# michaelneale/p2p-llm-tunnel

Measured on AMD Instinct MI355X. Metric: tunneled req/s + added p50 TTFT vs direct, mock-LLM SSE at 1/2/4/8 streams, higher is better.
Workload: dtype n/a

## Files before the change

p2p_llm_tunnel_amd/models/server.py:

```python
from __future__ import annotations

import argparse
import asyncio
import functools
import json
import os
import queue
import socket
import sys
import threading
import time
import uuid
from typing import NamedTuple

import torch


class Sampling:
    __slots__ = ("temperature", "top_k", "top_p", "seed")

    def __init__(self, temperature: float = 0.0, top_k: int = 0, top_p: float = 1.0, seed: int | None = None):
        self.temperature = float(temperature)
        self.top_k = int(top_k)
        self.top_p = float(top_p)
# ... 385 lines not shown
        self._pools = pools = []
        for r, row in enumerate(rows):
            s = self.slots[row.slot]
            if s["embed"]:
                if pools and pools[-1][0] == row.slot:
                    pools[-1][2] += 1
                else:
                    pools.append([row.slot, r, 1, row.pos == 0, None])
        max_seq = self.model.cfg.max_seq
        for row in rows:
            self.slots[row.slot]["pos"] += 1
            if not row.emit:
                self.prefill_tokens += 1
        done = []
        for r, row in enumerate(rows):
            if not row.emit:
                continue
            i = row.slot
            s = self.slots[i]
            s["gen"] += 1
            fin = s["gen"] >= s["req"].max_new or s["pos"] >= max_seq - 1
            emits.append((r, s["req"], fin, s["gen"] - 1))
            if fin:
                done.append(i)
        for pool in pools:
            s = self.slots[pool[0]]
            if s["pos"] >= len(s["ids"]):
                pool[4] = s["req"]
                done.append(pool[0])
        for i in done:
            self.slots[i] = None
        return rows, emits

    def _step_body(self, b: _StepBuf, n: int, run, sample_rows: int = 0, logprobs: bool = False):
        din = self._d_in[b.rows]
        din.copy_(b.h_in, non_blocking=True)
        d = din[:, :n]
        tok = torch.where(d[_DEC] != 0, self._d_last[d[_SLOT]], d[_TOK])
        ids, logits = run(tok, d[_POS].to(torch.int32), d[_SLOT].to(torch.int32))
        if sample_rows:
            from p2p_llm_tunnel_amd import ops
            ops.sample_(logits[:sample_rows], ids[:sample_rows], din[_SMP])
            if logprobs:
                ops.logprobs_(logits[:sample_rows], ids[:sample_rows], din[_LP], b.d_lp[:sample_rows],
                              b.d_lp_ids[:sample_rows])
                b.h_lp.copy_(b.d_lp, non_blocking=True)
                b.h_lp_ids.copy_(b.d_lp_ids, non_blocking=True)
        self._d_last.index_copy_(0, d[_REC], ids)
        b.h_out[:n].copy_(ids, non_blocking=True)

    def _capture(self, b: _StepBuf, emit_rows: int, post: int):
        from p2p_llm_tunnel_amd.models.tiny_llm import capture
        b.np[:] = 0
        b.np[_SLOT, :] = b.np[_REC, :] = self.model.scratch_slot
        run = functools.partial(self.model.step_rows, emit_rows=emit_rows)
        sample_rows = (emit_rows or b.rows) if post else 0
        graph, _ = capture(lambda: self._step_body(b, b.rows, run, sample_rows, post == 2), self.device)
        torch.cuda.synchronize(self.device)
        return graph

    def _launch(self, rows, emits) -> _StepBuf:
        n, scratch = len(rows), self.model.scratch_slot
        R = self.small_rows if self.use_graph and n <= self.small_rows else self.rows
        par = self._k % 2
        self._k += 1
        b = self._bufs[R][par]
        h = b.np
        h[_TOK, :n] = [r.token for r in rows]
        h[_POS, :n] = [r.pos for r in rows]
        h[_SLOT, :n] = [r.slot for r in rows]
        h[_DEC, :n] = [r.decode for r in rows]
        h[_REC, :n] = [r.slot if r.emit else scratch for r in rows]
        h[_SMP, :] = 0
        h[_LP, :] = 0
        post = 0
        for r, req, _, ctr in emits:
            if not req.sampling.greedy:
                h[_SMP, r] = req.sampling.column(ctr)
                post = max(post, 1)
            if req.logprobs is not None:
                h[_LP, r] = 1 + req.logprobs
                post = 2
        if n < R:
            h[_TOK, n:R] = h[_POS, n:R] = h[_DEC, n:R] = 0
            h[_SLOT, n:R] = h[_REC, n:R] = scratch
        b.n, b.emits = n, emits
        if self.use_graph:
            self._graphs[(R, par, post)].replay()
        else:
            rng = (min(r.pos for r in rows), max(r.pos for r in rows))
# ... 654 lines not shown
```

p2p_llm_tunnel_amd/models/tiny_llm.py:

```python
from __future__ import annotations

import math
from dataclasses import dataclass

import torch
import torch.nn.functional as F

from p2p_llm_tunnel_amd import ops


@dataclass(frozen=True)
class LlamaConfig:
    vocab: int = 32000
    dim: int = 1024
    n_layers: int = 4
    n_heads: int = 16
    n_kv_heads: int = 4
    head_dim: int = 64
    ffn: int = 2816
    max_seq: int = 2048
    eps: float = 1e-5
    rope_theta: float = 10000.0
    qk_norm: bool = False

# ... 111 lines not shown
            return torch.stack([torch.arange(n), torch.arange(n) + n], 1).flatten().to(self.device)

        heads = c.n_heads + 2 * c.n_kv_heads
        head_perm = (torch.arange(heads, device=self.device)[:, None] * c.head_dim
                     + pairs(c.head_dim // 2)[None, :]).flatten()
        ws = [self.embed, self.final_norm, fold(self.lm_head, self.final_norm)]
        for L in self.layers:
            wqkv = fold(L["wqkv"], L["attn_norm"])
            ws += [L["attn_norm"], wqkv.contiguous() if c.qk_norm else wqkv[head_perm].contiguous(), L["wo"],
                   L["ffn_norm"], fold(L["w_gate_up"], L["ffn_norm"])[pairs(c.ffn)].contiguous(), L["w_down"]]
            if c.qk_norm:
                ws += [L["q_norm"].contiguous(), L["k_norm"].contiguous()]
        return ws

    def fused_decoder(self) -> ops.FusedLlamaDecoder:
        if self._fused is None:
            c = self.cfg
            dims = ops.LlamaDims(vocab=c.vocab, dim=c.dim, n_layers=c.n_layers, H=c.n_heads, Hkv=c.n_kv_heads,
                                 D=c.head_dim, ffn=c.ffn, max_seq=c.max_seq, max_batch=self.max_batch + 1, eps=c.eps,
                                 theta=c.rope_theta, qk_norm=int(c.qk_norm))
            self._fused = ops.FusedLlamaDecoder(dims, self.fused_weights(), self.k_cache, self.v_cache)
        return self._fused

    def step_rows(self, tokens, pos, slots=None, emit_rows=0, pos_range=None):
        B = tokens.shape[0]
        if self.fused and B <= ops.MAX_ROWS:
            tokens, pos = tokens.contiguous(), pos.contiguous()
            slots = slots.contiguous() if slots is not None else None
            logits = torch.empty(B, self.cfg.vocab, dtype=torch.bfloat16, device=self.device)
            ids = torch.empty(B, dtype=torch.int64, device=self.device)
            self.fused_decoder().step(tokens, pos, logits, ids, slots, emit_rows)
            return ids, logits
        return self._decode_unfused(tokens, pos, pos_range or (0, self.cfg.max_seq - 1))

    def _decode_unfused(self, tokens, pos, pos_range):
        c = self.cfg
        B = tokens.shape[0]
        lens = pos + 1
        x = self.embed.index_select(0, tokens)
        h = ops.rmsnorm(x, self.layers[0]["attn_norm"], c.eps)
        residual = x
        for i, L in enumerate(self.layers):
            kc, vc = self.k_cache[i, :B], self.v_cache[i, :B]
            qkv = F.linear(h, L["wqkv"])
            if c.qk_norm:
                nq, nk = c.n_heads * c.head_dim, c.n_kv_heads * c.head_dim
                qn = ops.rmsnorm(qkv[:, :nq].reshape(-1, c.head_dim), L["q_norm"], c.eps).view(B, nq)
                kn = ops.rmsnorm(qkv[:, nq:nq + nk].reshape(-1, c.head_dim), L["k_norm"], c.eps).view(B, nk)
                qkv = torch.cat([qn, kn, qkv[:, nq + nk:]], 1)
            q = ops.rope_qkv_cache(qkv, pos, kc, vc, c.n_heads, c.n_kv_heads, c.head_dim, c.rope_theta,
                                   pos_range=pos_range)
            a = ops.decode_attention(q, kc, vc, lens, max_len=pos_range[1] + 1)
            o = F.linear(a.view(B, -1), L["wo"])
            h, residual = ops.rmsnorm(o, L["ffn_norm"], c.eps, residual=residual)
            m = F.linear(ops.silu_mul(F.linear(h, L["w_gate_up"])), L["w_down"])
            nxt = self.layers[i + 1]["attn_norm"] if i + 1 < len(self.layers) else self.final_norm
            h, residual = ops.rmsnorm(m, nxt, c.eps, residual=residual)
        logits = F.linear(h, self.lm_head)
        return ops.argmax(logits), logits

    def capture_graph(self, rows: int | None = None, emit_rows: int = 0):
        R = rows or (16 if self.fused else self.max_batch)
        g_tok = torch.zeros(R, dtype=torch.int64, device=self.device)
        g_pos = torch.zeros(R, dtype=torch.int32, device=self.device)
        g_slot = (torch.full((R,), self.scratch_slot, dtype=torch.int32, device=self.device)
                  if self.fused else None)
# ... 92 lines not shown
```

p2p_llm_tunnel_amd/ops/__init__.py:

```python
from __future__ import annotations

import ctypes
import math
import os

import torch

HERE = os.path.dirname(os.path.abspath(__file__))
_LIB = None


class LlamaDims(ctypes.Structure):
    _fields_ = [(n, ctypes.c_int) for n in ("vocab", "dim", "n_layers", "H", "Hkv", "D", "ffn", "max_seq",
                                           "max_batch")] + [("eps", ctypes.c_float), ("theta", ctypes.c_float),
                                                            ("qk_norm", ctypes.c_int)]


_INT = ctypes.c_int


class GemmPlan(ctypes.Structure):
    _fields_ = [(n, _INT) for n in ("epi", "nw", "tn", "um", "kpl", "grid_x", "grid_y", "ss_in", "M", "N", "K")]


class AttnPlan(ctypes.Structure):
    _fields_ = [(n, _INT) for n in ("D", "G", "slots", "stride", "grid_y")]


class StepPlan(ctypes.Structure):
    _fields_ = ([("rows", _INT), ("emit_rows", _INT)] +
                [(n, GemmPlan) for n in ("qkv_first", "qkv", "o", "gate_up", "down", "lm_head")] +
                [("attn", AttnPlan), ("am_parts", _INT), ("qk_norm_grid", _INT)])


def lib() -> ctypes.CDLL:
    global _LIB
    if _LIB is None:
        path = os.path.join(HERE, os.environ.get("P2PT_HIP_OPS_LIB", "_hip_ops.so"))
        if not os.path.exists(path):
            from . import build as _b
            _b.build()
        _LIB = ctypes.CDLL(path)
        vp, i, f = ctypes.c_void_p, ctypes.c_int, ctypes.c_float
        _LIB.p2pt_rmsnorm.argtypes = [vp, vp, vp, vp, vp, i, i, f, vp]
        _LIB.p2pt_silu_mul.argtypes = [vp, vp, i, i, vp]
        _LIB.p2pt_rope_qkv_cache.argtypes = [vp, vp, vp, vp, vp, i, i, i, i, i, f, vp]
        _LIB.p2pt_qk_norm_rope_cache.argtypes = [vp, vp, vp, vp, vp, vp, vp, vp, i, i, i, i, i, i, f, f, vp]
        _LIB.p2pt_decode_attention.argtypes = [vp, vp, vp, vp, vp, vp, i, i, i, i, i, i, i, f, vp]
        _LIB.p2pt_argmax.argtypes = [vp, vp, i, i, vp]
        _LIB.p2pt_skinny_gemm.argtypes = [vp, vp, vp, i, i, i, vp]
        _LIB.p2pt_sample.argtypes = [vp, vp, vp, i, i, i, vp]
        _LIB.p2pt_logprobs.argtypes = [vp, vp, vp, vp, vp, i, i, vp]
        _LIB.p2pt_kv_copy.argtypes = [vp, vp, i, i, i, i, i, ctypes.POINTER(ctypes.c_int), vp]
        _LIB.p2pt_max_kv_copy_jobs.argtypes = []
        _LIB.p2pt_embed_pool.argtypes = [vp, i, i, vp, vp, i, vp, i, f, i, ctypes.POINTER(ctypes.c_int), vp]
        _LIB.p2pt_max_embed_jobs.argtypes = []
        _LIB.p2pt_llama_ws_bytes.argtypes = [ctypes.POINTER(LlamaDims)]
        _LIB.p2pt_llama_ws_bytes.restype = ctypes.c_size_t
        szp = ctypes.POINTER(ctypes.c_size_t)
        _LIB.p2pt_llama_ws_layout.argtypes = [ctypes.POINTER(LlamaDims), szp, szp, i]
        _LIB.p2pt_llama_ws_layout.restype = ctypes.c_int
        _LIB.p2pt_llama_decode.argtypes = [ctypes.POINTER(LlamaDims), ctypes.POINTER(vp), vp, vp, vp, vp, vp, i, i,
                                           vp, ctypes.c_size_t, vp, vp, vp]
        _LIB.p2pt_llama_plan.argtypes = [ctypes.POINTER(LlamaDims), i, i, ctypes.POINTER(StepPlan)]
        _LIB.p2pt_attn_span.argtypes = [i, i]
        _LIB.p2pt_max_rows.argtypes = []
        _LIB.p2pt_skinny_bench.argtypes = [vp, vp, vp, i, i, i, i, i, i, vp]
        _LIB.p2pt_attn_bench.argtypes = [vp, vp, vp, vp, i, i, i, i, i, vp, vp, vp, vp, i, vp]
        for fn in ("p2pt_rmsnorm", "p2pt_silu_mul", "p2pt_rope_qkv_cache", "p2pt_decode_attention", "p2pt_argmax",
                   "p2pt_skinny_gemm", "p2pt_llama_decode", "p2pt_sample", "p2pt_logprobs", "p2pt_llama_plan", "p2pt_attn_span",
                   "p2pt_max_rows", "p2pt_skinny_bench", "p2pt_attn_bench", "p2pt_kv_copy", "p2pt_max_kv_copy_jobs",
                   "p2pt_embed_pool", "p2pt_max_embed_jobs", "p2pt_qk_norm_rope_cache"):
            getattr(_LIB, fn).restype = ctypes.c_int
        if _LIB.p2pt_max_rows() != MAX_ROWS:
            raise RuntimeError(f"MAX_ROWS = {MAX_ROWS}, but {path} was built for {_LIB.p2pt_max_rows()} rows")
        if _LIB.p2pt_max_kv_copy_jobs() != MAX_KV_COPY_JOBS:
            raise RuntimeError(f"MAX_KV_COPY_JOBS = {MAX_KV_COPY_JOBS}, but {path} was built for "
                               f"{_LIB.p2pt_max_kv_copy_jobs()} jobs")
        if _LIB.p2pt_max_embed_jobs() != MAX_EMBED_JOBS:
            raise RuntimeError(f"MAX_EMBED_JOBS = {MAX_EMBED_JOBS}, but {path} was built for "
                               f"{_LIB.p2pt_max_embed_jobs()} jobs")
    return _LIB


MAX_ROWS = 64
MAX_KV_COPY_JOBS = 8
MAX_EMBED_JOBS = 16
MAX_TOP_LOGPROBS = 20


def step_plan(dims: LlamaDims, B: int, emit_rows: int = 0) -> StepPlan:
    plan = StepPlan()
    if lib().p2pt_llama_plan(ctypes.byref(dims), B, emit_rows, ctypes.byref(plan)) != 0:
        raise ValueError("dims or row count not supported by the fused decode kernels")
    return plan


def attn_span(length: int, slots: int) -> int:
    return lib().p2pt_attn_span(length, slots)


def loaded_path() -> str:
    return lib()._name


# ... 162 lines not shown
        raise ValueError("lens exceed cache capacity")
    nsplit = max(1, math.ceil(max_len / chunk))
    ws = torch.empty(B * H * nsplit * (D + 2), dtype=torch.float32, device=q.device)
    out = torch.empty_like(q)
    scale = 1.0 / math.sqrt(D) if scale is None else scale
    _ok(lib().p2pt_decode_attention(_p(q), _p(k_cache), _p(v_cache), _p(lens), _p(out), _p(ws), B, H, Hkv, D, Smax,
                                    nsplit, chunk, scale, _stream(q)), "decode_attention")
    return out


def argmax(logits: torch.Tensor) -> torch.Tensor:
    _check(logits, torch.bfloat16, "logits")
    if logits.dim() != 2:
        raise ValueError("logits must be [B, V]")
    B, V = logits.shape
    out = torch.empty(B, dtype=torch.int64, device=logits.device)
    _ok(lib().p2pt_argmax(_p(logits), _p(out), B, V, _stream(logits)), "argmax")
    return out


def sample_(logits: torch.Tensor, ids: torch.Tensor, params: torch.Tensor) -> torch.Tensor:
    _check(logits, torch.bfloat16, "logits")
    _check(ids, torch.int64, "ids", logits.device)
    _check(params, torch.int64, "params", logits.device)
    if logits.dim() != 2 or ids.shape != (logits.shape[0],) or params.dim() != 2 or params.shape[0] != 5:
        raise ValueError("need logits [B, V], ids [B], params [5, >= B]")
    B, V = logits.shape
    if params.shape[1] < B:
        raise ValueError("params need a column per row")
    _ok(lib().p2pt_sample(_p(logits), _p(ids), _p(params), B, params.shape[1], V, _stream(logits)), "sample")
    return ids


def logprobs_(logits: torch.Tensor, ids: torch.Tensor, want: torch.Tensor, out_lp: torch.Tensor,
              out_ids: torch.Tensor) -> None:
    _check(logits, torch.bfloat16, "logits")
    _check(ids, torch.int64, "ids", logits.device)
    _check(want, torch.int64, "want", logits.device)
    _check(out_lp, torch.float32, "out_lp", logits.device)
    _check(out_ids, torch.int32, "out_ids", logits.device)
    if logits.dim() != 2 or ids.shape != (logits.shape[0],) or want.dim() != 1:
        raise ValueError("need logits [B, V], ids [B], want [>= B]")
    B, V = logits.shape
    if B < 1 or V < 32:
        raise ValueError("need B >= 1 and V >= 32")
    if want.shape[0] < B:
        raise ValueError("want needs an entry per row")
    if out_lp.shape != (B, MAX_TOP_LOGPROBS + 1) or out_ids.shape != (B, MAX_TOP_LOGPROBS):
        raise ValueError(f"need out_lp [B, {MAX_TOP_LOGPROBS + 1}] and out_ids [B, {MAX_TOP_LOGPROBS}]")
    _ok(lib().p2pt_logprobs(_p(logits), _p(ids), _p(want), _p(out_lp), _p(out_ids), B, V, _stream(logits)),
        "logprobs")


def kv_copy_(k_cache: torch.Tensor, v_cache: torch.Tensor, jobs) -> None:
    _check(k_cache, torch.bfloat16, "k_cache")
    _check(v_cache, torch.bfloat16, "v_cache", k_cache.device)
    if k_cache.dim() != 5 or v_cache.dim() != 5:
        raise ValueError("caches must be [n_layers, n_slots, max_seq, Hkv, D]")
    if k_cache.shape != v_cache.shape:
        raise ValueError(f"cache shapes differ: {tuple(k_cache.shape)} and {tuple(v_cache.shape)}")
    L, n_slots, max_seq, Hkv, D = k_cache.shape
    if (Hkv * D * 2) % 16 or Hkv * D == 0 or L == 0 or max_seq == 0:
        raise ValueError("a cache row (Hkv * D bf16) must be a non-empty multiple of 16 bytes")
    jobs = list(jobs)
    if not 1 <= len(jobs) <= MAX_KV_COPY_JOBS:
        raise ValueError(f"need 1..{MAX_KV_COPY_JOBS} jobs, got {len(jobs)}")
# ... 101 lines not shown


class FusedLlamaDecoder:

    def __init__(self, dims: LlamaDims, weights: list, k_cache: torch.Tensor, v_cache: torch.Tensor):
        self.dims = dims
        dev = k_cache.device
        for i, t in enumerate(weights):
            _check(t, torch.bfloat16, f"weight[{i}]", dev)
        L, Bmax, S, Hkv, D = k_cache.shape
        if (L, Bmax, S, Hkv, D) != (dims.n_layers, dims.max_batch, dims.max_seq, dims.Hkv, dims.D):
            raise ValueError("cache shape does not match dims")
        _check(k_cache, torch.bfloat16, "k_cache", dev)
        _check(v_cache, torch.bfloat16, "v_cache", dev)
        per_layer = 8 if dims.qk_norm else 6
        if len(weights) != 3 + per_layer * dims.n_layers:
            raise ValueError(f"weight table: embed, final_norm, lm_head, then {per_layer} per layer "
                             "(wqkv, w_gate_up and lm_head with the preceding norm weight folded in"
                             + ("; q_norm and k_norm last)" if dims.qk_norm else ")"))
        if dims.qk_norm:
            for L in range(dims.n_layers):
                for j in (6, 7):
                    if weights[3 + 8 * L + j].shape != (dims.D,):
                        raise ValueError(f"layer {L}: q_norm and k_norm must be ({dims.D},)")
        nbytes = lib().p2pt_llama_ws_bytes(ctypes.byref(dims))
        if nbytes == 0:
            raise ValueError("model dims not supported by the fused decode kernels")
        self.weights = weights
        self._wptr = (ctypes.c_void_p * len(weights))(*[t.data_ptr() for t in weights])
        self.ws = torch.zeros(nbytes, dtype=torch.uint8, device=dev)
        self.k_cache, self.v_cache = k_cache, v_cache
        self.device = dev
        self._resid = None

    _WS_BUFFERS = (("resid", torch.bfloat16), ("q", torch.bfloat16), ("attn", torch.bfloat16), ("h", torch.bfloat16),
                   ("ss", torch.float32), ("part_o", torch.float32), ("part_ml", torch.float32),
                   ("am_val", torch.float32), ("am_idx", torch.int32), ("counters", torch.int32),
                   ("qkv", torch.bfloat16))

    def workspace_views(self) -> dict:
        d = self.dims
        n = len(self._WS_BUFFERS)
        off, cnt = (ctypes.c_size_t * n)(), (ctypes.c_size_t * n)()
        if lib().p2pt_llama_ws_layout(ctypes.byref(d), off, cnt, n) != n:
            raise RuntimeError("workspace layout: buffer list out of step with decode_fused.hip")
        views = {}
        for (name, dtype), o, c in zip(self._WS_BUFFERS, off, cnt):
            size = torch.empty(0, dtype=dtype).element_size()
            if o % size or o + c * size > self.ws.numel():
                raise RuntimeError(f"workspace layout: {name} lies outside the workspace")
            views[name] = self.ws[o:o + c * size].view(dtype)
        M = MAX_ROWS
        shapes = {"resid": (M, d.dim), "q": (M, d.H, d.D), "attn": (M, d.H * d.D), "h": (M, d.ffn), "ss": (-1, M),
                  "part_o": (M, d.H, -1, d.D), "part_ml": (M, d.H, -1, 2), "am_val": (-1, M), "am_idx": (-1, M),
                  "counters": (M * d.H,), "qkv": (M if d.qk_norm else 0, (d.H + 2 * d.Hkv) * d.D)}
        return {name: v.view(*shapes[name]) for name, v in views.items()}

    def embed_pool(self, acc: torch.Tensor, out: torch.Tensor, jobs) -> None:
        if self._resid is None:
            self._resid = self.workspace_views()["resid"]
        embed_pool_(self._resid, self.weights[1], acc, out, jobs, self.dims.eps)

    def step(self, tokens: torch.Tensor, pos: torch.Tensor, logits: torch.Tensor, ids: torch.Tensor,
             slots: torch.Tensor | None = None, emit_rows: int = 0) -> None:
        d = self.dims
        _check(tokens, torch.int64, "tokens", self.device)
        _check(pos, torch.int32, "pos", self.device)
        _check(logits, torch.bfloat16, "logits", self.device)
        _check(ids, torch.int64, "ids", self.device)
        B = tokens.shape[0]
        if slots is not None:
            _check(slots, torch.int32, "slots", self.device)
            if slots.shape != (B,):
                raise ValueError("slots must be [B]")
        limit = MAX_ROWS if slots is not None else min(MAX_ROWS, d.max_batch)
        if not 0 <= emit_rows <= B:
            raise ValueError("emit_rows must be in 0..B")
        if not 1 <= B <= limit or pos.shape != (B,) or ids.shape != (B,):
            raise ValueError(f"rows must be 1..{limit} with matching pos/ids")
        if logits.shape != (B, d.vocab):
            raise ValueError("logits must be [B, vocab]")
        _ok(lib().p2pt_llama_decode(ctypes.byref(d), self._wptr, _p(self.k_cache), _p(self.v_cache), _p(tokens),
                                    _p(pos), _p(slots), B, emit_rows, _p(self.ws), self.ws.numel(), _p(logits),
                                    _p(ids), _stream(tokens)), "llama_decode")
```

p2p_llm_tunnel_amd/ops/decode_fused.hip:

```cpp
#include "decode_fused_kernels.h"

namespace {

struct LlamaDims {
  int vocab, dim, n_layers, H, Hkv, D, ffn, max_seq, max_batch;
  float eps, theta;
  int qk_norm;
};

constexpr int kTnResid = 1, kTnStore = 2;
constexpr int kCUs = 256;
constexpr int kMaxKpl = 2;

struct GemmPlan {
  int epi, nw, tn, um, kpl;
  int grid_x, grid_y;
  int ss_in;
  int M, N, K;
};
struct AttnPlan {
  int D, G;
  int slots;
  int stride;
  int grid_y;
};
struct StepPlan {
  int rows, emit_rows;
  GemmPlan qkv_first, qkv, o, gate_up, down, lm_head;
  AttnPlan attn;
  int am_parts;
  int qk_norm_grid;
};

// ... 188 lines not shown
    case 128 * 16 + 8: return go(k_attn<128, 8>);
  }
  return hipErrorInvalidValue;
}

hipError_t launch_qknorm(int grid_x, int rows, int D, const QkNormArgs& a, hipStream_t s) {
  if (grid_x <= 0 || rows <= 0 || grid_x * qknorm_heads_per_wg(D) < a.H + 2 * a.Hkv) return hipErrorInvalidValue;
  const dim3 g(grid_x, rows), b(kQkNormWaves * 64);
  switch (D) {
    case 64: hipLaunchKernelGGL(k_qknorm_rope<64>, g, b, 0, s, a); break;
    case 128: hipLaunchKernelGGL(k_qknorm_rope<128>, g, b, 0, s, a); break;
    default: return hipErrorInvalidValue;
  }
  return hipGetLastError();
}

bool dims_ok(const LlamaDims& d) {
  if (d.D != 64 && d.D != 128) return false;
  if (d.qk_norm != 0 && d.qk_norm != 1) return false;
  const size_t dim = size_t(d.dim), ffn = size_t(d.ffn), hd = size_t(d.H) * d.D;
  const size_t gemm_bytes[] = {size_t(d.vocab) * dim * 2, size_t(d.H + 2 * d.Hkv) * d.D * dim * 2,
                               2 * ffn * dim * 2, dim * hd * 2, dim * ffn * 2};
  for (size_t b : gemm_bytes)
    if (b >= kOob) return false;
  if (d.H % d.Hkv || (d.H / d.Hkv != 1 && d.H / d.Hkv != 2 && d.H / d.Hkv != 4 && d.H / d.Hkv != 8)) return false;
  if (d.dim % 32 || (d.H * d.D) % 32 || d.ffn % 32) return false;
  if (d.dim % (16 * kTnResid) || d.vocab % (16 * kTnStore) || d.ffn % 16) return false;
  if (d.max_batch <= 0 || d.max_seq <= 0 || d.n_layers <= 0) return false;
  return true;
}

bool rows_ok(int B) { return B > 0 && B <= kMaxM; }

}

extern "C" {

size_t p2pt_llama_ws_bytes(const LlamaDims* d) {
  if (!dims_ok(*d)) return 0;
  return carve(*d, nullptr).bytes;
}

int p2pt_llama_ws_layout(const LlamaDims* d, size_t* off, size_t* count, int n) {
  if (!dims_ok(*d) || n < WS_NBUF) return 0;
  const WsLayout l = ws_layout(*d);
  for (int b = 0; b < WS_NBUF; b++) {
    off[b] = l.off[b];
    count[b] = l.count[b];
  }
  return WS_NBUF;
}

int p2pt_llama_plan(const LlamaDims* d, int B, int emit_rows, StepPlan* out) {
  if (!dims_ok(*d) || !rows_ok(B)) return int(hipErrorInvalidValue);
  *out = plan_step(*d, B, emit_rows);
  return 0;
}

int p2pt_attn_span(int len, int slots) { return len > 0 && slots > 0 ? attn_span(len, unsigned(slots)) : 0; }

int p2pt_max_rows() { return kMaxM; }

int p2pt_llama_decode(const LlamaDims* dp, const void* const* w, void* k_cache, void* v_cache, const int64_t* tokens,
                      const int* pos, const int* slots, int B, int emit_rows, void* ws, size_t ws_bytes, void* logits,
                      int64_t* ids, void* stream) {
  const LlamaDims d = *dp;
  if (!dims_ok(d) || !rows_ok(B) || (!slots && B > d.max_batch)) return int(hipErrorInvalidValue);
  const Workspace W = carve(d, static_cast<uint8_t*>(ws));
  if (ws_bytes < W.bytes) return int(hipErrorInvalidValue);
  const StepPlan P = plan_step(d, B, emit_rows);
  auto s = static_cast<hipStream_t>(stream);
  const size_t layer_cache = size_t(d.max_batch) * d.max_seq * d.Hkv * d.D;
  hipError_t e;
  auto failed = [&](hipError_t r) { return (e = r) != hipSuccess; };

  hipLaunchKernelGGL(k_embed, dim3(B), dim3(256), 0, s, static_cast<const uint16_t*>(w[0]), tokens, W.resid, W.ss,
                     d.dim, d.vocab);
  if (failed(hipGetLastError())) return int(e);
  for (int L = 0; L < d.n_layers; L++) {
    const void* const* wl = w + 3 + (d.qk_norm ? 8 : 6) * L;
    uint16_t* kc = static_cast<uint16_t*>(k_cache) + L * layer_cache;
    uint16_t* vc = static_cast<uint16_t*>(v_cache) + L * layer_cache;
    const GemmPlan& qkv = L ? P.qkv : P.qkv_first;
    const GemmArgs to_qkv = d.qk_norm
                                ? gemm(W.resid, wl[1]) + norm(W.ss, qkv.ss_in, d.eps) + store(W.qkv)
                                : gemm(W.resid, wl[1]) + norm(W.ss, qkv.ss_in, d.eps) + rope(d, pos, slots, W.q, kc, vc);
    const GemmArgs to_o = gemm(W.attn, wl[2]) + resid(W.resid, W.ss);
    const GemmArgs to_gate_up = gemm(W.resid, wl[4]) + norm(W.ss, P.gate_up.ss_in, d.eps) + store(W.h);
    const GemmArgs to_down = gemm(W.h, wl[5]) + resid(W.resid, W.ss);
    if (failed(launch(qkv, to_qkv, s))) return int(e);
    if (P.qk_norm_grid) {
      const QkNormArgs qn{W.qkv, static_cast<const uint16_t*>(wl[6]), static_cast<const uint16_t*>(wl[7]), pos, slots,
                          d.max_batch, W.q, kc, vc, d.H, d.Hkv, d.max_seq, d.eps, log2f(d.theta)};
      if (failed(launch_qknorm(P.qk_norm_grid, B, d.D, qn, s))) return int(e);
    }
    if (failed(launch_attn(P.attn, W.q, kc, vc, pos, slots, d.max_batch, W.part_o, W.part_ml, W.counters, W.attn, d.H,
                           d.Hkv, d.max_seq, s)))
      return int(e);
    if (failed(launch(P.o, to_o, s))) return int(e);
    if (failed(launch(P.gate_up, to_gate_up, s))) return int(e);
    if (failed(launch(P.down, to_down, s))) return int(e);
  }
  const GemmArgs to_logits =
      gemm(W.resid, w[2]) + norm(W.ss, P.lm_head.ss_in, d.eps) + argmax(logits, W.am_val, W.am_idx);
  if (failed(launch(P.lm_head, to_logits, s))) return int(e);
  hipLaunchKernelGGL(k_argmax_merge, dim3(P.emit_rows), dim3(256), 0, s, W.am_val, W.am_idx, P.am_parts, ids);
  return int(hipGetLastError());
}

int p2pt_skinny_gemm(const void* x, const void* w, void* out, int M, int N, int K, void* stream) {
  if (!rows_ok(M) || N % 32 || K <= 0 || K % 32) return int(hipErrorInvalidValue);
  const GemmPlan p = plan_gemm(EPI_STORE, 2, M, N, K);
  return int(launch(p, gemm(x, w) + store(out), static_cast<hipStream_t>(stream)));
}

int p2pt_qk_norm_rope_cache(const void* qkv, const int* pos, const int* slots, const void* q_weight,
                            const void* k_weight, void* q, void* k_cache, void* v_cache, int B, int H, int Hkv, int D,
                            int Smax, int nslots, float eps, float theta, void* stream) {
  if (!rows_ok(B) || (D != 64 && D != 128) || H <= 0 || Hkv <= 0 || Smax <= 0 || nslots <= 0)
    return int(hipErrorInvalidValue);
  if ((!slots && B > nslots) || !(theta > 0.f)) return int(hipErrorInvalidValue);
  const QkNormArgs a{static_cast<const uint16_t*>(qkv), static_cast<const uint16_t*>(q_weight),
                     static_cast<const uint16_t*>(k_weight), pos, slots, nslots, static_cast<uint16_t*>(q),
                     static_cast<uint16_t*>(k_cache), static_cast<uint16_t*>(v_cache), H, Hkv, Smax, eps, log2f(theta)};
  const int per_wg = qknorm_heads_per_wg(D);
  return int(launch_qknorm((H + 2 * Hkv + per_wg - 1) / per_wg, B, D, a, static_cast<hipStream_t>(stream)));
}

int p2pt_attn_bench(const void* q, const void* kc, const void* vc, const int* pos, int B, int H, int Hkv, int D,
                    int Smax, float* part_o, float* part_ml, unsigned* counters, void* out, int reps, void* stream) {
  if (!rows_ok(B) || Hkv <= 0 || H % Hkv || Smax <= 0 || reps <= 0) return int(hipErrorInvalidValue);
  const AttnPlan p = plan_attn(B, H, Hkv, D, Smax);
  for (int r = 0; r < reps; r++) {
    hipError_t e = launch_attn(p, q, kc, vc, pos, nullptr, B, part_o, part_ml, counters, out, H, Hkv, Smax,
                               static_cast<hipStream_t>(stream));
    if (e != hipSuccess) return int(e);
  }
  return 0;
}

// ... 15 lines not shown
```

p2p_llm_tunnel_amd/ops/decode_fused_kernels.h:

```cpp
#pragma once
#include "bf16_common.h"

#include <algorithm>

namespace {

using namespace p2pt_gpu;

constexpr int kMaxM = 64;

typedef short frag8 __attribute__((ext_vector_type(8)));
typedef float frag4 __attribute__((ext_vector_type(4)));

enum Epi : int { EPI_STORE = 0, EPI_ROPE = 1, EPI_SILU = 2, EPI_RESID = 3, EPI_ARGMAX = 4 };

struct GemmArgs {
  const uint16_t* x;
  const uint16_t* w;
  int M, N, K;
  const float* ss_part;
  int ss_parts;
  float eps;
  uint16_t* out;
  float* ss_out;
// ... 262 lines not shown
        sincosf(float(p) * inv_freq, &sn, &cs);
        const float x1 = second ? other : mine, x2 = second ? mine : other;
        const float o = second ? x2 * cs + x1 * sn : x1 * cs - x2 * sn;
        uint16_t* dst = head < a.H ? a.q_out + (size_t(m) * a.H + head) * a.D
                                   : a.kc + ((size_t(sl) * a.Smax + p) * a.Hkv + (head - a.H)) * a.D;
        dst[d] = uint16_t(f2bf_bits(o));
      } else {
        a.vc[((size_t(sl) * a.Smax + p) * a.Hkv + (head - a.H - a.Hkv)) * a.D + d] = uint16_t(f2bf_bits(mine));
      }
    }
  } else if constexpr (EPI == EPI_RESID) {
    float sq[4] = {0.f, 0.f, 0.f, 0.f};
#pragma unroll
    for (int t = 0; t < TN; t++) {
      const int n = tile_col<TN>(bx, t, c, cwl);
#pragma unroll
      for (int r = 0; r < 4; r++) {
        const int m = mrow0 + r;
        if (m >= a.M || !col_ok) continue;
        const float nv = bf_round(rprev[t][r] + bf_round(v[t][r]));
        a.out[size_t(m) * a.N + n] = uint16_t(f2bf_bits(nv));
        sq[r] += nv * nv;
      }
    }
#pragma unroll
    for (int r = 0; r < 4; r++) {
      sq[r] = row16_sum(sq[r]);
      if (c == 0) a.ss_out[bx * kMaxM + mrow0 + r] = sq[r];
    }
  }
}

__global__ __launch_bounds__(256) void k_argmax_merge(const float* __restrict__ am_val, const int* __restrict__ am_idx,
                                                      int parts, int64_t* __restrict__ ids) {
  const int m = blockIdx.x;
  float b = -INFINITY;
  int i = 0x7fffffff;
  for (int p0 = threadIdx.x; p0 < parts; p0 += 8 * 256) {
    float pv[8];
    int pi[8];
#pragma unroll
    for (int j = 0; j < 8; j++) {
      const int p = p0 + j * 256;
      pv[j] = p < parts ? am_val[p * kMaxM + m] : -INFINITY;
      pi[j] = p < parts ? am_idx[p * kMaxM + m] : 0x7fffffff;
    }
#pragma unroll
    for (int j = 0; j < 8; j++)
      if (pv[j] > b || (pv[j] == b && pi[j] < i)) {
        b = pv[j];
        i = pi[j];
      }
  }
  wave_argmax(b, i);
  __shared__ float sb[4];
  __shared__ int si[4];
  if ((threadIdx.x & 63) == 0) {
    sb[threadIdx.x >> 6] = b;
    si[threadIdx.x >> 6] = i;
  }
  __syncthreads();
  if (threadIdx.x == 0) {
    for (int w = 1; w < 4; w++)
      if (sb[w] > b || (sb[w] == b && si[w] < i)) {
        b = sb[w];
        i = si[w];
      }
    ids[m] = i == 0x7fffffff ? 0 : i;
  }
}

__global__ __launch_bounds__(256) void k_embed(const uint16_t* __restrict__ embed, const int64_t* __restrict__ tok,
                                               uint16_t* __restrict__ resid, float* __restrict__ ss_out, int dim,
                                               int vocab) {
  const int b = blockIdx.x;
  int64_t t = tok[b];
  t = t < 0 ? 0 : (t >= vocab ? vocab - 1 : t);
  const uint4* src = reinterpret_cast<const uint4*>(embed + size_t(t) * dim);
  uint4* dst = reinterpret_cast<uint4*>(resid + size_t(b) * dim);
  float ss = 0.f;
  for (int i = threadIdx.x; i < dim / 8; i += 256) {
    const uint4 v = src[i];
    dst[i] = v;
    float f[8];
    unpack8(v, f);
#pragma unroll
    for (int j = 0; j < 8; j++) ss += f[j] * f[j];
  }
  __shared__ float red[4];
  ss = wave_sum(ss);
  if ((threadIdx.x & 63) == 0) red[threadIdx.x >> 6] = ss;
  __syncthreads();
  if (threadIdx.x == 0) ss_out[b] = red[0] + red[1] + red[2] + red[3];
}

struct QkNormArgs {
  const uint16_t* qkv;
  const uint16_t* gq;
  const uint16_t* gk;
  const int* pos;
  const int* slot;
  int nslots;
  uint16_t* q_out;
  uint16_t* kc;
  uint16_t* vc;
  int H, Hkv, Smax;
  float eps, log2_theta;
};

// ... 277 lines not shown
```

p2p_llm_tunnel_amd/ops/sample.hip:

```cpp
#include "bf16_common.h"

namespace {

using namespace p2pt_gpu;

constexpr int kThreads = 1024, kWaves = kThreads / 64;

__device__ __forceinline__ uint32_t okey(float f) {
  uint32_t u = __float_as_uint(f);
  return (u & 0x80000000u) ? ~u : (u | 0x80000000u);
}

__device__ __forceinline__ uint64_t mix64(uint64_t z) {
  z = (z ^ (z >> 30)) * 0xBF58476D1CE4E5B9ull;
  z = (z ^ (z >> 27)) * 0x94D049BB133111EBull;
  return z ^ (z >> 31);
}

__device__ __forceinline__ float gumbel(uint64_t seed, uint64_t ctr, uint32_t i) {
  uint64_t h = mix64(seed + mix64(ctr * 0x9E3779B97F4A7C15ull + i + 1));
  double u = (double(h >> 11) + 0.5) * (1.0 / 9007199254740992.0);
  return float(-log(-log(u)));
}

// ... 26 lines not shown
#pragma unroll
  for (int q = 0; q < 4; q++) {
    v[q] = hist[255 - 4 * lane - q];
    s += v[q];
  }
  T incl = s;
#pragma unroll
  for (int d = 1; d < 64; d <<= 1) {
    T o = __shfl_up(incl, d, 64);
    if (lane >= d) incl += o;
  }
  const T excl = incl - s;
  const bool hit = excl < need && incl >= need;
  const uint64_t b = __ballot(hit);
  const int first = b ? __ffsll((unsigned long long)b) - 1 : 63;
  if (lane == first) {
    T run = excl;
    int dg = 255 - 4 * lane - 3;
    T ab = run;
#pragma unroll
    for (int q = 0; q < 4; q++) {
      if (run + v[q] >= need || q == 3) {
        dg = 255 - 4 * lane - q;
        ab = run;
        break;
      }
      run += v[q];
    }
    *digit_out = dg;
    *above_out = ab;
  }
}

__global__ __launch_bounds__(kThreads) void k_sample(const uint16_t* __restrict__ logits, int64_t* __restrict__ ids,
                                                     const int64_t* __restrict__ params, int ld, int V) {
  const int row = blockIdx.x;
  const int B = ld;
  const float T = __uint_as_float(uint32_t(params[row]));
  if (!(T >= 1e-4f)) return;
  int64_t k = params[B + row];
  float p = __uint_as_float(uint32_t(params[2 * B + row]));
  const uint64_t seed = uint64_t(params[3 * B + row]), ctr = uint64_t(params[4 * B + row]);
  if (k <= 0 || k > V) k = V;
  if (!(p > 0.f && p < 1.f)) p = 1.f;
  const float invT = 1.0f / T;
  const uint16_t* lr = logits + size_t(row) * V;

  __shared__ float red[kWaves];
  __shared__ uint32_t hist_u[256];
  __shared__ float hist_f[256];
  __shared__ int s_digit;
  __shared__ uint32_t s_above_u;
  __shared__ float s_above_f;
  __shared__ float s_best[kWaves];
  __shared__ int s_bi[kWaves];

  float m = -INFINITY;
  for (int i = threadIdx.x; i < V; i += kThreads) m = fmaxf(m, bf2f(lr[i]) * invT);
  m = block_max(m, red);

  uint32_t kth = 0;
  if (k < V) {
    uint32_t prefix = 0, mask = 0, need = uint32_t(k);
    for (int shift = 24; shift >= 0; shift -= 8) {
      for (int d = threadIdx.x; d < 256; d += kThreads) hist_u[d] = 0;
      __syncthreads();
      for (int i = threadIdx.x; i < V; i += kThreads) {
        const uint32_t key = okey(bf2f(lr[i]) * invT);
        if ((key & mask) == prefix) atomicAdd(&hist_u[(key >> shift) & 0xFF], 1u);
      }
      __syncthreads();
      if (threadIdx.x < 64) find_bucket<uint32_t>(hist_u, need, &s_digit, &s_above_u);
// ... 21 lines not shown
      for (int i = threadIdx.x; i < V; i += kThreads) {
        const float zi = bf2f(lr[i]) * invT;
        const uint32_t key = okey(zi);
        if (key >= kth && (key & mask) == prefix) atomicAdd(&hist_f[(key >> shift) & 0xFF], __expf(zi - m));
      }
      __syncthreads();
      if (threadIdx.x < 64) find_bucket<float>(hist_f, need, &s_digit, &s_above_f);
      __syncthreads();
      need -= s_above_f;
      prefix |= uint32_t(s_digit) << shift;
      mask |= 0xFFu << shift;
      __syncthreads();
    }
    pth = prefix;
  }
  const uint32_t cut = kth > pth ? kth : pth;

  float best = -INFINITY;
  int bi = 0x7fffffff;
  for (int i = threadIdx.x; i < V; i += kThreads) {
    const float zi = bf2f(lr[i]) * invT;
    if (okey(zi) < cut) continue;
    am_take(best, bi, zi + gumbel(seed, ctr, uint32_t(i)), i);
  }
  wave_argmax(best, bi);
  if ((threadIdx.x & 63) == 0) {
    s_best[threadIdx.x >> 6] = best;
    s_bi[threadIdx.x >> 6] = bi;
  }
  __syncthreads();
  if (threadIdx.x == 0) {
    for (int w = 1; w < kWaves; w++) am_take(best, bi, s_best[w], s_bi[w]);
    if (bi != 0x7fffffff) ids[row] = bi;
  }
}

}

extern "C" {

int p2pt_sample(const void* logits, int64_t* ids, const int64_t* params, int B, int ld, int V, void* stream) {
  if (B <= 0 || V <= 0 || ld < B) return int(hipErrorInvalidValue);
  hipLaunchKernelGGL(k_sample, dim3(B), dim3(kThreads), 0, static_cast<hipStream_t>(stream),
                     static_cast<const uint16_t*>(logits), ids, params, ld, V);
  return int(hipGetLastError());
}

}
```

Baseline: 15.96.

## Fold token select, index casts and last-token record into fused decode kernels

Adds a staged decode entry point where the embed kernel reads token, position, slot and decode flags directly from the staged input tensor. It selects the previous token on device and writes the int32 position and slot arrays itself, replacing the separate torch.where, gather and cast ops. The argmax-merge and sample kernels now also write each row's id into the last-token buffer, removing the index_copy_ launch. This trims several small kernel launches from each captured step, at the cost of more native plumbing and new bounds-clamping logic.

```diff
diff --git a/p2p_llm_tunnel_amd/models/server.py b/p2p_llm_tunnel_amd/models/server.py
--- a/p2p_llm_tunnel_amd/models/server.py
+++ b/p2p_llm_tunnel_amd/models/server.py
@@ -441,30 +441,44 @@
             self.slots[i] = None
         return rows, emits
 
-    def _step_body(self, b: _StepBuf, n: int, run, sample_rows: int = 0, logprobs: bool = False):
+    def _step_body(self, b: _StepBuf, n: int, run, sample_rows: int = 0, logprobs: bool = False,
+                   staged_emit: int | None = None):
+        from p2p_llm_tunnel_amd import ops
         din = self._d_in[b.rows]
         din.copy_(b.h_in, non_blocking=True)
-        d = din[:, :n]
-        tok = torch.where(d[_DEC] != 0, self._d_last[d[_SLOT]], d[_TOK])
-        ids, logits = run(tok, d[_POS].to(torch.int32), d[_SLOT].to(torch.int32))
+        native = staged_emit is not None
+        if native:
+            ids, logits = self.model.step_staged(din, (_TOK, _POS, _SLOT, _DEC, _REC), self._d_last, n, staged_emit,
+                                                 record=not sample_rows)
+        else:
+            d = din[:, :n]
+            tok = torch.where(d[_DEC] != 0, self._d_last[d[_SLOT]], d[_TOK])
+            ids, logits = run(tok, d[_POS].to(torch.int32), d[_SLOT].to(torch.int32))
         if sample_rows:
-            from p2p_llm_tunnel_amd import ops
-            ops.sample_(logits[:sample_rows], ids[:sample_rows], din[_SMP])
+            if native:
+                ops.sample_rows_(logits[:sample_rows], ids[:sample_rows], din[_SMP], din[_REC], self._d_last)
+            else:
+                ops.sample_(logits[:sample_rows], ids[:sample_rows], din[_SMP])
             if logprobs:
                 ops.logprobs_(logits[:sample_rows], ids[:sample_rows], din[_LP], b.d_lp[:sample_rows],
                               b.d_lp_ids[:sample_rows])
                 b.h_lp.copy_(b.d_lp, non_blocking=True)
                 b.h_lp_ids.copy_(b.d_lp_ids, non_blocking=True)
-        self._d_last.index_copy_(0, d[_REC], ids)
+        if not native:
+            self._d_last.index_copy_(0, d[_REC], ids)
         b.h_out[:n].copy_(ids, non_blocking=True)
 
     def _capture(self, b: _StepBuf, emit_rows: int, post: int):
+        from p2p_llm_tunnel_amd import ops
         from p2p_llm_tunnel_amd.models.tiny_llm import capture
         b.np[:] = 0
         b.np[_SLOT, :] = b.np[_REC, :] = self.model.scratch_slot
         run = functools.partial(self.model.step_rows, emit_rows=emit_rows)
         sample_rows = (emit_rows or b.rows) if post else 0
-        graph, _ = capture(lambda: self._step_body(b, b.rows, run, sample_rows, post == 2), self.device)
+        staged = getattr(self.model, "fused", False) and callable(getattr(self.model, "step_staged", None)) \
+            and b.rows <= ops.MAX_ROWS
+        graph, _ = capture(lambda: self._step_body(b, b.rows, run, sample_rows, post == 2,
+                                                   emit_rows if staged else None), self.device)
         torch.cuda.synchronize(self.device)
         return graph
 
diff --git a/p2p_llm_tunnel_amd/models/tiny_llm.py b/p2p_llm_tunnel_amd/models/tiny_llm.py
--- a/p2p_llm_tunnel_amd/models/tiny_llm.py
+++ b/p2p_llm_tunnel_amd/models/tiny_llm.py
@@ -167,6 +167,14 @@
             self.fused_decoder().step(tokens, pos, logits, ids, slots, emit_rows)
             return ids, logits
         return self._decode_unfused(tokens, pos, pos_range or (0, self.cfg.max_seq - 1))
+
+    def step_staged(self, staged, rows, last, B, emit_rows=0, record=True):
+        if not self.fused:
+            raise ValueError("step_staged needs the fused path")
+        logits = torch.empty(B, self.cfg.vocab, dtype=torch.bfloat16, device=self.device)
+        ids = torch.empty(B, dtype=torch.int64, device=self.device)
+        self.fused_decoder().step_staged(staged, rows, last, logits, ids, B, emit_rows, record)
+        return ids, logits
 
     def _decode_unfused(self, tokens, pos, pos_range):
         c = self.cfg
diff --git a/p2p_llm_tunnel_amd/ops/__init__.py b/p2p_llm_tunnel_amd/ops/__init__.py
--- a/p2p_llm_tunnel_amd/ops/__init__.py
+++ b/p2p_llm_tunnel_amd/ops/__init__.py
@@ -31,6 +31,11 @@
     _fields_ = ([("rows", _INT), ("emit_rows", _INT)] +
                 [(n, GemmPlan) for n in ("qkv_first", "qkv", "o", "gate_up", "down", "lm_head")] +
                 [("attn", AttnPlan), ("am_parts", _INT), ("qk_norm_grid", _INT)])
+
+
+class StagedIn(ctypes.Structure):
+    _fields_ = [("data", ctypes.c_void_p), ("ld", _INT), ("rows", _INT)] + \
+               [(n, _INT) for n in ("tok", "pos", "slot", "dec", "rec")]
 
 
 def lib() -> ctypes.CDLL:
@@ -62,6 +67,10 @@
         _LIB.p2pt_llama_ws_layout.restype = ctypes.c_int
         _LIB.p2pt_llama_decode.argtypes = [ctypes.POINTER(LlamaDims), ctypes.POINTER(vp), vp, vp, vp, vp, vp, i, i,
                                            vp, ctypes.c_size_t, vp, vp, vp]
+        _LIB.p2pt_llama_decode_rows.argtypes = [ctypes.POINTER(LlamaDims), ctypes.POINTER(vp), vp, vp,
+                                                ctypes.POINTER(StagedIn), vp, i, i, vp, vp, i, i, vp, ctypes.c_size_t,
+                                                vp, vp, vp]
+        _LIB.p2pt_sample_rows.argtypes = [vp, vp, vp, i, i, i, vp, vp, i, vp]
         _LIB.p2pt_llama_plan.argtypes = [ctypes.POINTER(LlamaDims), i, i, ctypes.POINTER(StepPlan)]
         _LIB.p2pt_attn_span.argtypes = [i, i]
         _LIB.p2pt_max_rows.argtypes = []
@@ -70,7 +79,8 @@
         for fn in ("p2pt_rmsnorm", "p2pt_silu_mul", "p2pt_rope_qkv_cache", "p2pt_decode_attention", "p2pt_argmax",
                    "p2pt_skinny_gemm", "p2pt_llama_decode", "p2pt_sample", "p2pt_logprobs", "p2pt_llama_plan", "p2pt_attn_span",
                    "p2pt_max_rows", "p2pt_skinny_bench", "p2pt_attn_bench", "p2pt_kv_copy", "p2pt_max_kv_copy_jobs",
-                   "p2pt_embed_pool", "p2pt_max_embed_jobs", "p2pt_qk_norm_rope_cache"):
+                   "p2pt_embed_pool", "p2pt_max_embed_jobs", "p2pt_qk_norm_rope_cache", "p2pt_llama_decode_rows",
+                   "p2pt_sample_rows"):
             getattr(_LIB, fn).restype = ctypes.c_int
         if _LIB.p2pt_max_rows() != MAX_ROWS:
             raise RuntimeError(f"MAX_ROWS = {MAX_ROWS}, but {path} was built for {_LIB.p2pt_max_rows()} rows")
@@ -299,6 +309,25 @@
     return ids
 
 
+def sample_rows_(logits: torch.Tensor, ids: torch.Tensor, params: torch.Tensor, rec: torch.Tensor,
+                 last: torch.Tensor) -> torch.Tensor:
+    _check(logits, torch.bfloat16, "logits")
+    _check(ids, torch.int64, "ids", logits.device)
+    _check(params, torch.int64, "params", logits.device)
+    _check(rec, torch.int64, "rec", logits.device)
+    _check(last, torch.int64, "last", logits.device)
+    if logits.dim() != 2 or ids.shape != (logits.shape[0],) or params.dim() != 2 or params.shape[0] != 5:
+        raise ValueError("need logits [B, V], ids [B], params [5, >= B]")
+    B, V = logits.shape
+    if params.shape[1] < B:
+        raise ValueError("params need a column per row")
+    if rec.dim() != 1 or rec.shape[0] < B or last.dim() != 1 or last.shape[0] < 1:
+        raise ValueError("need rec [>= B] and last [n >= 1]")
+    _ok(lib().p2pt_sample_rows(_p(logits), _p(ids), _p(params), B, params.shape[1], V, _p(rec), _p(last),
+                               last.shape[0], _stream(logits)), "sample_rows")
+    return ids
+
+
 def logprobs_(logits: torch.Tensor, ids: torch.Tensor, want: torch.Tensor, out_lp: torch.Tensor,
               out_ids: torch.Tensor) -> None:
     _check(logits, torch.bfloat16, "logits")
@@ -466,6 +495,7 @@
         self.k_cache, self.v_cache = k_cache, v_cache
         self.device = dev
         self._resid = None
+        self.rows32 = torch.zeros(2, MAX_ROWS, dtype=torch.int32, device=dev)
 
     _WS_BUFFERS = (("resid", torch.bfloat16), ("q", torch.bfloat16), ("attn", torch.bfloat16), ("h", torch.bfloat16),
                    ("ss", torch.float32), ("part_o", torch.float32), ("part_ml", torch.float32),
@@ -517,3 +547,28 @@
         _ok(lib().p2pt_llama_decode(ctypes.byref(d), self._wptr, _p(self.k_cache), _p(self.v_cache), _p(tokens),
                                     _p(pos), _p(slots), B, emit_rows, _p(self.ws), self.ws.numel(), _p(logits),
                                     _p(ids), _stream(tokens)), "llama_decode")
+
+    def step_staged(self, staged: torch.Tensor, rows, last: torch.Tensor, logits: torch.Tensor, ids: torch.Tensor,
+                    B: int, emit_rows: int = 0, record: bool = True) -> None:
+        d = self.dims
+        _check(staged, torch.int64, "staged", self.device)
+        _check(last, torch.int64, "last", self.device)
+        _check(logits, torch.bfloat16, "logits", self.device)
+        _check(ids, torch.int64, "ids", self.device)
+        if staged.dim() != 2 or last.dim() != 1 or last.shape[0] < 1:
+            raise ValueError("need staged [n_rows, ld] and last [n >= 1]")
+        n_rows, ld = staged.shape
+        rows = tuple(rows)
+        if len(rows) != 5 or not all(isinstance(r, int) and not isinstance(r, bool) and 0 <= r < n_rows for r in rows):
+            raise ValueError(f"rows must be five row indices (tok, pos, slot, dec, rec) in [0, {n_rows})")
+        if isinstance(B, bool) or not isinstance(B, int) or not 1 <= B <= min(MAX_ROWS, ld):
+            raise ValueError(f"B must be in 1..{min(MAX_ROWS, ld)}")
+        if not 0 <= emit_rows <= B:
+            raise ValueError("emit_rows must be in 0..B")
+        if ids.shape != (B,) or logits.shape != (B, d.vocab):
+            raise ValueError("need ids [B] and logits [B, vocab]")
+        st = StagedIn(staged.data_ptr(), ld, n_rows, *rows)
+        _ok(lib().p2pt_llama_decode_rows(ctypes.byref(d), self._wptr, _p(self.k_cache), _p(self.v_cache),
+                                         ctypes.byref(st), _p(last), last.shape[0], int(bool(record)),
+                                         _p(self.rows32[0]), _p(self.rows32[1]), B, emit_rows, _p(self.ws),
+                                         self.ws.numel(), _p(logits), _p(ids), _stream(staged)), "llama_decode_rows")
diff --git a/p2p_llm_tunnel_amd/ops/decode_fused.hip b/p2p_llm_tunnel_amd/ops/decode_fused.hip
--- a/p2p_llm_tunnel_amd/ops/decode_fused.hip
+++ b/p2p_llm_tunnel_amd/ops/decode_fused.hip
@@ -1,4 +1,6 @@
 #include "decode_fused_kernels.h"
+
+#include <initializer_list>
 
 namespace {
 
@@ -253,50 +255,39 @@
 
 bool rows_ok(int B) { return B > 0 && B <= kMaxM; }
 
-}
-
-extern "C" {
-
-size_t p2pt_llama_ws_bytes(const LlamaDims* d) {
-  if (!dims_ok(*d)) return 0;
-  return carve(*d, nullptr).bytes;
-}
-
-int p2pt_llama_ws_layout(const LlamaDims* d, size_t* off, size_t* count, int n) {
-  if (!dims_ok(*d) || n < WS_NBUF) return 0;
-  const WsLayout l = ws_layout(*d);
-  for (int b = 0; b < WS_NBUF; b++) {
-    off[b] = l.off[b];
-    count[b] = l.count[b];
-  }
-  return WS_NBUF;
-}
-
-int p2pt_llama_plan(const LlamaDims* d, int B, int emit_rows, StepPlan* out) {
-  if (!dims_ok(*d) || !rows_ok(B)) return int(hipErrorInvalidValue);
-  *out = plan_step(*d, B, emit_rows);
-  return 0;
-}
-
-int p2pt_attn_span(int len, int slots) { return len > 0 && slots > 0 ? attn_span(len, unsigned(slots)) : 0; }
-
-int p2pt_max_rows() { return kMaxM; }
-
-int p2pt_llama_decode(const LlamaDims* dp, const void* const* w, void* k_cache, void* v_cache, const int64_t* tokens,
-                      const int* pos, const int* slots, int B, int emit_rows, void* ws, size_t ws_bytes, void* logits,
-                      int64_t* ids, void* stream) {
-  const LlamaDims d = *dp;
-  if (!dims_ok(d) || !rows_ok(B) || (!slots && B > d.max_batch)) return int(hipErrorInvalidValue);
+struct StagedIn {
+  const int64_t* in;
+  int ld, rows;
+  int tok, pos, slot, dec, rec;
+};
+
+struct StepRows {
+  const int64_t* tokens;
+  StagedRows staged;
+  const int* pos;
+  const int* slots;
+  const int64_t* rec;
+  int64_t* last;
+  int nlast;
+};
+
+int run_step(const LlamaDims& d, const void* const* w, void* k_cache, void* v_cache, const StepRows& r, int B,
+             int emit_rows, void* ws, size_t ws_bytes, void* logits, int64_t* ids, void* stream) {
   const Workspace W = carve(d, static_cast<uint8_t*>(ws));
   if (ws_bytes < W.bytes) return int(hipErrorInvalidValue);
   const StepPlan P = plan_step(d, B, emit_rows);
   auto s = static_cast<hipStream_t>(stream);
   const size_t layer_cache = size_t(d.max_batch) * d.max_seq * d.Hkv * d.D;
+  const int *pos = r.pos, *slots = r.slots;
   hipError_t e;
-  auto failed = [&](hipError_t r) { return (e = r) != hipSuccess; };
-
-  hipLaunchKernelGGL(k_embed, dim3(B), dim3(256), 0, s, static_cast<const uint16_t*>(w[0]), tokens, W.resid, W.ss,
-                     d.dim, d.vocab);
+  auto failed = [&](hipError_t rc) { return (e = rc) != hipSuccess; };
+
+  if (r.staged.in)
+    hipLaunchKernelGGL(k_embed<true>, dim3(B), dim3(256), 0, s, static_cast<const uint16_t*>(w[0]), r.tokens, r.staged,
+                       W.resid, W.ss, d.dim, d.vocab);
+  else
+    hipLaunchKernelGGL(k_embed<false>, dim3(B), dim3(256), 0, s, static_cast<const uint16_t*>(w[0]), r.tokens,
+                       r.staged, W.resid, W.ss, d.dim, d.vocab);
   if (failed(hipGetLastError())) return int(e);
   for (int L = 0; L < d.n_layers; L++) {
     const void* const* wl = w + 3 + (d.qk_norm ? 8 : 6) * L;
@@ -325,8 +316,63 @@
   const GemmArgs to_logits =
       gemm(W.resid, w[2]) + norm(W.ss, P.lm_head.ss_in, d.eps) + argmax(logits, W.am_val, W.am_idx);
   if (failed(launch(P.lm_head, to_logits, s))) return int(e);
-  hipLaunchKernelGGL(k_argmax_merge, dim3(P.emit_rows), dim3(256), 0, s, W.am_val, W.am_idx, P.am_parts, ids);
+  hipLaunchKernelGGL(k_argmax_merge, dim3(P.emit_rows), dim3(256), 0, s, W.am_val, W.am_idx, P.am_parts, ids, r.rec,
+                     r.last, r.nlast);
   return int(hipGetLastError());
+}
+
+}
+
+extern "C" {
+
+size_t p2pt_llama_ws_bytes(const LlamaDims* d) {
+  if (!dims_ok(*d)) return 0;
+  return carve(*d, nullptr).bytes;
+}
+
+int p2pt_llama_ws_layout(const LlamaDims* d, size_t* off, size_t* count, int n) {
+  if (!dims_ok(*d) || n < WS_NBUF) return 0;
+  const WsLayout l = ws_layout(*d);
+  for (int b = 0; b < WS_NBUF; b++) {
+    off[b] = l.off[b];
+    count[b] = l.count[b];
+  }
+  return WS_NBUF;
+}
+
+int p2pt_llama_plan(const LlamaDims* d, int B, int emit_rows, StepPlan* out) {
+  if (!dims_ok(*d) || !rows_ok(B)) return int(hipErrorInvalidValue);
+  *out = plan_step(*d, B, emit_rows);
+  return 0;
+}
+
+int p2pt_attn_span(int len, int slots) { return len > 0 && slots > 0 ? attn_span(len, unsigned(slots)) : 0; }
+
+int p2pt_max_rows() { return kMaxM; }
+
+int p2pt_llama_decode(const LlamaDims* dp, const void* const* w, void* k_cache, void* v_cache, const int64_t* tokens,
+                      const int* pos, const int* slots, int B, int emit_rows, void* ws, size_t ws_bytes, void* logits,
+                      int64_t* ids, void* stream) {
+  const LlamaDims d = *dp;
+  if (!dims_ok(d) || !rows_ok(B) || (!slots && B > d.max_batch)) return int(hipErrorInvalidValue);
+  StepRows r{};
+  r.tokens = tokens, r.pos = pos, r.slots = slots;
+  return run_step(d, w, k_cache, v_cache, r, B, emit_rows, ws, ws_bytes, logits, ids, stream);
+}
+
+int p2pt_llama_decode_rows(const LlamaDims* dp, const void* const* w, void* k_cache, void* v_cache, const StagedIn* st,
+                           int64_t* last, int nlast, int record, int* pos32, int* slot32, int B, int emit_rows,
+                           void* ws, size_t ws_bytes, void* logits, int64_t* ids, void* stream) {
+  const LlamaDims d = *dp;
+  if (!dims_ok(d) || !rows_ok(B)) return int(hipErrorInvalidValue);
+  if (!st || !st->in || !last || !pos32 || !slot32 || nlast <= 0 || st->ld < B) return int(hipErrorInvalidValue);
+  for (int row : {st->tok, st->pos, st->slot, st->dec, st->rec})
+    if (row < 0 || row >= st->rows) return int(hipErrorInvalidValue);
+  StepRows r{};
+  r.staged = {st->in, st->ld, st->tok, st->pos, st->slot, st->dec, last, nlast, pos32, slot32};
+  r.pos = pos32, r.slots = slot32;
+  if (record) r.rec = st->in + size_t(st->rec) * st->ld, r.last = last, r.nlast = nlast;
+  return run_step(d, w, k_cache, v_cache, r, B, emit_rows, ws, ws_bytes, logits, ids, stream);
 }
 
 int p2pt_skinny_gemm(const void* x, const void* w, void* out, int M, int N, int K, void* stream) {
diff --git a/p2p_llm_tunnel_amd/ops/decode_fused_kernels.h b/p2p_llm_tunnel_amd/ops/decode_fused_kernels.h
--- a/p2p_llm_tunnel_amd/ops/decode_fused_kernels.h
+++ b/p2p_llm_tunnel_amd/ops/decode_fused_kernels.h
@@ -318,7 +318,9 @@
 }
 
 __global__ __launch_bounds__(256) void k_argmax_merge(const float* __restrict__ am_val, const int* __restrict__ am_idx,
-                                                      int parts, int64_t* __restrict__ ids) {
+                                                      int parts, int64_t* __restrict__ ids,
+                                                      const int64_t* __restrict__ rec, int64_t* __restrict__ last,
+                                                      int nlast) {
   const int m = blockIdx.x;
   float b = -INFINITY;
   int i = 0x7fffffff;
@@ -352,15 +354,44 @@
         b = sb[w];
         i = si[w];
       }
-    ids[m] = i == 0x7fffffff ? 0 : i;
-  }
-}
-
+    const int64_t id = i == 0x7fffffff ? 0 : i;
+    ids[m] = id;
+    if (rec) {
+      const int64_t r = rec[m];
+      if (r >= 0 && r < nlast) last[r] = id;
+    }
+  }
+}
+
+struct StagedRows {
+  const int64_t* in;
+  int ld;
+  int tok, pos, slot, dec;
+  const int64_t* last;
+  int nlast;
+  int* pos32;
+  int* slot32;
+};
+
+template <bool STAGED>
 __global__ __launch_bounds__(256) void k_embed(const uint16_t* __restrict__ embed, const int64_t* __restrict__ tok,
-                                               uint16_t* __restrict__ resid, float* __restrict__ ss_out, int dim,
-                                               int vocab) {
+                                               StagedRows st, uint16_t* __restrict__ resid,
+                                               float* __restrict__ ss_out, int dim, int vocab) {
   const int b = blockIdx.x;
-  int64_t t = tok[b];
+  int64_t t;
+  if constexpr (STAGED) {
+    const int64_t sl = st.in[size_t(st.slot) * st.ld + b];
+    if (st.in[size_t(st.dec) * st.ld + b] != 0)
+      t = st.last[sl < 0 ? 0 : (sl >= st.nlast ? st.nlast - 1 : sl)];
+    else
+      t = st.in[size_t(st.tok) * st.ld + b];
+    if (threadIdx.x == 0) {
+      st.pos32[b] = int(st.in[size_t(st.pos) * st.ld + b]);
+      st.slot32[b] = int(sl);
+    }
+  } else {
+    t = tok[b];
+  }
   t = t < 0 ? 0 : (t >= vocab ? vocab - 1 : t);
   const uint4* src = reinterpret_cast<const uint4*>(embed + size_t(t) * dim);
   uint4* dst = reinterpret_cast<uint4*>(resid + size_t(b) * dim);
diff --git a/p2p_llm_tunnel_amd/ops/sample.hip b/p2p_llm_tunnel_amd/ops/sample.hip
--- a/p2p_llm_tunnel_amd/ops/sample.hip
+++ b/p2p_llm_tunnel_amd/ops/sample.hip
@@ -82,12 +82,23 @@
   }
 }
 
+__device__ __forceinline__ void record(const int64_t* rec, int64_t* last, int nlast, int row, int64_t id) {
+  if (!rec) return;
+  const int64_t r = rec[row];
+  if (r >= 0 && r < nlast) last[r] = id;
+}
+
 __global__ __launch_bounds__(kThreads) void k_sample(const uint16_t* __restrict__ logits, int64_t* __restrict__ ids,
-                                                     const int64_t* __restrict__ params, int ld, int V) {
+                                                     const int64_t* __restrict__ params, int ld, int V,
+                                                     const int64_t* __restrict__ rec, int64_t* __restrict__ last,
+                                                     int nlast) {
   const int row = blockIdx.x;
   const int B = ld;
   const float T = __uint_as_float(uint32_t(params[row]));
-  if (!(T >= 1e-4f)) return;
+  if (!(T >= 1e-4f)) {
+    if (threadIdx.x == 0) record(rec, last, nlast, row, ids[row]);
+    return;
+  }
   int64_t k = params[B + row];
   float p = __uint_as_float(uint32_t(params[2 * B + row]));
   const uint64_t seed = uint64_t(params[3 * B + row]), ctr = uint64_t(params[4 * B + row]);
@@ -175,6 +186,7 @@
   if (threadIdx.x == 0) {
     for (int w = 1; w < kWaves; w++) am_take(best, bi, s_best[w], s_bi[w]);
     if (bi != 0x7fffffff) ids[row] = bi;
+    record(rec, last, nlast, row, bi != 0x7fffffff ? int64_t(bi) : ids[row]);
   }
 }
 
@@ -182,11 +194,17 @@
 
 extern "C" {
 
+int p2pt_sample_rows(const void* logits, int64_t* ids, const int64_t* params, int B, int ld, int V, const int64_t* rec,
+                     int64_t* last, int nlast, void* stream) {
+  if (B <= 0 || V <= 0 || ld < B) return int(hipErrorInvalidValue);
+  if (rec && (!last || nlast <= 0)) return int(hipErrorInvalidValue);
+  hipLaunchKernelGGL(k_sample, dim3(B), dim3(kThreads), 0, static_cast<hipStream_t>(stream),
+                     static_cast<const uint16_t*>(logits), ids, params, ld, V, rec, last, nlast);
+  return int(hipGetLastError());
+}
+
 int p2pt_sample(const void* logits, int64_t* ids, const int64_t* params, int B, int ld, int V, void* stream) {
-  if (B <= 0 || V <= 0 || ld < B) return int(hipErrorInvalidValue);
-  hipLaunchKernelGGL(k_sample, dim3(B), dim3(kThreads), 0, static_cast<hipStream_t>(stream),
-                     static_cast<const uint16_t*>(logits), ids, params, ld, V);
-  return int(hipGetLastError());
-}
-
-}
+  return p2pt_sample_rows(logits, ids, params, B, ld, V, nullptr, nullptr, 0, stream);
+}
+
+}
```

Result: no change. 15.97, median of 4 (+0.0%).
